# NightShade99/Self-Supervised-Vision

Hardware: NVIDIA B200
Metric: ntxent_fwd_bwd_samples_per_s (higher is better)
Workload: dtype f16

## Files before the change

### self-supervised-vision_b200/csrc/common.cuh

```cuda
#pragma once
#include <cuda.h>
#include <cuda_runtime.h>
#include <cuda_bf16.h>
#include <stdint.h>

#define SSVB_LOG2E 1.4426950408889634f
#define SSVB_LN2 0.6931471805599453f

namespace ssvb {

__device__ __forceinline__ uint32_t smem_u32(const void* p) {
  return static_cast<uint32_t>(__cvta_generic_to_shared(p));
}
__device__ __forceinline__ float ex2f(float x) {
  float y;
  asm("ex2.approx.ftz.f32 %0, %1;" : "=f"(y) : "f"(x));
  return y;
}
__device__ __forceinline__ float lg2f(float x) {
  float y;
  asm("lg2.approx.ftz.f32 %0, %1;" : "=f"(y) : "f"(x));
  return y;
}
__device__ __forceinline__ uint32_t pack_bf16x2(float lo, float hi) {
// ... 183 lines not shown
               "n"(NCOLS)
               : "memory");
  asm volatile("tcgen05.relinquish_alloc_permit.cta_group::1.sync.aligned;" ::: "memory");
}
template <int NCOLS>
__device__ __forceinline__ void tmem_dealloc(uint32_t taddr) {
  asm volatile("tcgen05.dealloc.cta_group::1.sync.aligned.b32 %0, %1;" ::"r"(taddr), "n"(NCOLS) : "memory");
}
__device__ __forceinline__ void tc_fence_before() {
  asm volatile("tcgen05.fence::before_thread_sync;" ::: "memory");
}
__device__ __forceinline__ void tc_fence_after() {
  asm volatile("tcgen05.fence::after_thread_sync;" ::: "memory");
}
__device__ __forceinline__ void umma_commit(uint64_t* bar) {
  asm volatile("tcgen05.commit.cta_group::1.mbarrier::arrive::one.shared::cluster.b64 [%0];" ::"r"(smem_u32(bar))
               : "memory");
}

__device__ __forceinline__ uint64_t make_smem_desc(uint32_t saddr, uint32_t lbo_bytes, uint32_t sbo_bytes) {
  uint64_t d = 0;
  d |= static_cast<uint64_t>((saddr & 0x3FFFFu) >> 4);
  d |= static_cast<uint64_t>((lbo_bytes >> 4) & 0x3FFFu) << 16;
  d |= static_cast<uint64_t>((sbo_bytes >> 4) & 0x3FFFu) << 32;
  d |= static_cast<uint64_t>(1) << 46;
  d |= static_cast<uint64_t>(2) << 61;
  return d;
}
__device__ __forceinline__ uint64_t desc_kmajor(uint32_t saddr) { return make_smem_desc(saddr, 16, 1024); }
__device__ __forceinline__ uint64_t desc_mnmajor(uint32_t saddr, uint32_t lbo_bytes) {
  return make_smem_desc(saddr, lbo_bytes, 1024);
}

__host__ __device__ constexpr uint32_t make_idesc(int M, int N, int a_mn_major, int b_mn_major, int ab_fmt = 1) {
  return (1u << 4) | (static_cast<uint32_t>(ab_fmt) << 7) | (static_cast<uint32_t>(ab_fmt) << 10) |
         (static_cast<uint32_t>(a_mn_major) << 15) |
         (static_cast<uint32_t>(b_mn_major) << 16) | (static_cast<uint32_t>(N >> 3) << 17) |
         (static_cast<uint32_t>(M >> 4) << 24);
}

__device__ __forceinline__ void umma_ss(uint32_t d_tmem, uint64_t adesc, uint64_t bdesc, uint32_t idesc,
                                        uint32_t accumulate) {
  asm volatile(
      "{\n\t.reg .pred p;\n\tsetp.ne.b32 p, %4, 0;\n\t"
      "tcgen05.mma.cta_group::1.kind::f16 [%0], %1, %2, %3, p;\n\t}\n"
      ::"r"(d_tmem), "l"(adesc), "l"(bdesc), "r"(idesc), "r"(accumulate)
      : "memory");
}
__device__ __forceinline__ void umma_ts(uint32_t d_tmem, uint32_t a_tmem, uint64_t bdesc, uint32_t idesc,
                                        uint32_t accumulate) {
  asm volatile(
      "{\n\t.reg .pred p;\n\tsetp.ne.b32 p, %4, 0;\n\t"
      "tcgen05.mma.cta_group::1.kind::f16 [%0], [%1], %2, %3, p;\n\t}\n"
      ::"r"(d_tmem), "r"(a_tmem), "l"(bdesc), "r"(idesc), "r"(accumulate)
      : "memory");
}

__device__ __forceinline__ void tmem_ld_x32(uint32_t taddr, uint32_t (&v)[32]) {
  asm volatile(
      "tcgen05.ld.sync.aligned.32x32b.x32.b32 "
      "{%0, %1, %2, %3, %4, %5, %6, %7, %8, %9, %10, %11, %12, %13, %14, %15, "
      "%16, %17, %18, %19, %20, %21, %22, %23, %24, %25, %26, %27, %28, %29, %30, %31}, [%32];"
      : "=r"(v[0]), "=r"(v[1]), "=r"(v[2]), "=r"(v[3]), "=r"(v[4]), "=r"(v[5]), "=r"(v[6]), "=r"(v[7]),
        "=r"(v[8]), "=r"(v[9]), "=r"(v[10]), "=r"(v[11]), "=r"(v[12]), "=r"(v[13]), "=r"(v[14]), "=r"(v[15]),
        "=r"(v[16]), "=r"(v[17]), "=r"(v[18]), "=r"(v[19]), "=r"(v[20]), "=r"(v[21]), "=r"(v[22]), "=r"(v[23]),
        "=r"(v[24]), "=r"(v[25]), "=r"(v[26]), "=r"(v[27]), "=r"(v[28]), "=r"(v[29]), "=r"(v[30]), "=r"(v[31])
      : "r"(taddr)
      : "memory");
}
__device__ __forceinline__ void tmem_ld_wait() { asm volatile("tcgen05.wait::ld.sync.aligned;" ::: "memory"); }
__device__ __forceinline__ void tmem_st_x16(uint32_t taddr, const uint32_t (&v)[16]) {
  asm volatile(
      "tcgen05.st.sync.aligned.32x32b.x16.b32 [%0], "
      "{%1, %2, %3, %4, %5, %6, %7, %8, %9, %10, %11, %12, %13, %14, %15, %16};"
      ::"r"(taddr), "r"(v[0]), "r"(v[1]), "r"(v[2]), "r"(v[3]), "r"(v[4]), "r"(v[5]), "r"(v[6]), "r"(v[7]),
        "r"(v[8]), "r"(v[9]), "r"(v[10]), "r"(v[11]), "r"(v[12]), "r"(v[13]), "r"(v[14]), "r"(v[15])
      : "memory");
}
__device__ __forceinline__ void tmem_st_wait() { asm volatile("tcgen05.wait::st.sync.aligned;" ::: "memory"); }

__device__ __forceinline__ void pdl_wait() { asm volatile("griddepcontrol.wait;" ::: "memory"); }
__device__ __forceinline__ void pdl_launch_dependents() { asm volatile("griddepcontrol.launch_dependents;" ::: "memory"); }

__device__ __forceinline__ void red_add_v4(float* addr, float a, float b, float c, float d) {
  asm volatile("red.global.add.v4.f32 [%0], {%1, %2, %3, %4};" ::"l"(addr), "f"(a), "f"(b), "f"(c), "f"(d)
               : "memory");
}

}
```

### self-supervised-vision_b200/csrc/ntxent.cu

```cuda
#include "sim_host.cuh"

using namespace ssvb;

namespace {

struct NtxPlan {
  int64_t n_glob, m, mpad, d, dpad;
  int mode;
  int normalize;
  float c, shift;
  float prescale;
  float wscale;
  float pos_c;
};

int make_plan(NtxPlan& pl, int64_t n_glob, int64_t d, int normalize, float temperature) {
  if (n_glob <= 0 || d <= 0 || !(temperature > 0.f)) return SSVB_ERR_INVALID;
  if (d % 4) return SSVB_ERR_ALIGNMENT;
  if (d > 256) return SSVB_ERR_UNSUPPORTED;
  if (2 * n_glob > (1 << 30)) return SSVB_ERR_UNSUPPORTED;
  pl.n_glob = n_glob;
  pl.m = 2 * n_glob;
  pl.mpad = sim_mpad(pl.m);
  pl.d = d;
// ... 163 lines not shown

int ssvb_ntxent_fwd(const float* zi, const float* zj, int64_t n, int64_t d, int64_t ld_zi, int64_t ld_zj,
                    int normalize, float temperature, float* loss, void* saved, void* workspace,
                    size_t workspace_bytes, void* stream) {
  SSVB_TRY(check_device_sm100());
  NtxPlan pl;
  SSVB_TRY(make_plan(pl, n, d, normalize, temperature));
  SSVB_TRY(check_rows(zi, ld_zi));
  SSVB_TRY(check_rows(zj, ld_zj));
  if (!loss || !saved || !workspace) return SSVB_ERR_INVALID;
  if (workspace_bytes < ssvb_ntxent_workspace_bytes(n, d)) return SSVB_ERR_WORKSPACE;
  cudaStream_t s = static_cast<cudaStream_t>(stream);
  SavedLayout sv = saved_layout(saved, pl.mpad, pl.dpad);
  WsLayout ws = ws_layout(workspace, pl.m, ceil_div(pl.m, 128), pl.m, pl.dpad);

  if (pl.mpad > pl.m)
    SSVB_CUDA(cudaMemsetAsync(sv.zhat + pl.m * pl.dpad, 0, (pl.mpad - pl.m) * pl.dpad * sizeof(__nv_bfloat16), s));
  {
    const int wpb = 8;
    pair_prep_kernel<<<static_cast<unsigned>(ceil_div(n, wpb)), wpb * 32, 0, s>>>(
        zi, zj, static_cast<int>(n), static_cast<int>(d), ld_zi, ld_zj, normalize, normalize ? 1 : 0, sv.zhat,
        sv.zhat + n * pl.dpad,
        static_cast<int>(pl.dpad), sv.inv_norm, sv.inv_norm + n, ws.pos, ws.pos + n, -1, pl.prescale, ws.counter);
    SSVB_LAUNCH_CHECK();
  }
  SimParams p;
  fill_sim_params_rows(p, pl, 1, pl.m, 0, 0);
  p.part_m = ws.part_m;
  p.part_l = ws.part_l;
  p.part_stride = static_cast<int>(round_up(pl.m, 256));
  int nparts;
  if (pl.mode == SIM_NTX_FIXED && pl.dpad <= 128) {
    const int ncol = plan_sym(p);
    p.colpart = ws.part_l + static_cast<size_t>(4 * p.nchunks) * p.part_stride;
    nparts = 4 * p.nchunks + ncol;
    SSVB_TRY(launch_sim_fwd_sym(sv.zhat, pl.mpad, pl.dpad, p, s));
  } else {
    plan_chunks(p, sim_fwd_bn(pl.dpad), sim_fwd_min_tiles(pl.dpad));
    nparts = 4 * p.nchunks;
    SSVB_TRY(launch_sim_fwd(pl.mode, sv.zhat, pl.mpad, sv.zhat, pl.mpad, pl.dpad, p, s));
  }
  {
    const unsigned grid = static_cast<unsigned>(ceil_div(pl.m, 256));
    const float scale = 1.f / static_cast<float>(pl.m);
    if (pl.mode == SIM_NTX_FIXED)
      lse_finalize_kernel<SIM_NTX_FIXED><<<grid, 256, 0, s>>>(ws.part_m, ws.part_l, nparts, p.part_stride,
                                                            static_cast<int>(pl.m), ws.pos, pl.c, pl.shift,
                                                            sv.stat, nullptr, ws.block_sums, ws.counter, scale, loss,
                                                            nullptr, nullptr, 0, 0, pl.wscale);
    else
      lse_finalize_kernel<SIM_NTX_ONLINE><<<grid, 256, 0, s>>>(ws.part_m, ws.part_l, nparts, p.part_stride,
                                                             static_cast<int>(pl.m), ws.pos, pl.c, pl.shift,
                                                             sv.stat, nullptr, ws.block_sums, ws.counter, scale, loss);
    SSVB_LAUNCH_CHECK();
    if (pl.mpad > pl.m) {
      const float padv = pl.mode == SIM_NTX_FIXED ? 0.f : 1e30f;
      fill_kernel<<<static_cast<unsigned>(ceil_div(pl.mpad - pl.m, 256)), 256, 0, s>>>(sv.stat + pl.m,
                                                                                       pl.mpad - pl.m, padv);
      SSVB_LAUNCH_CHECK();
    }
  }
  return SSVB_OK;
}

int ssvb_ntxent_bwd(const float* zi, const float* zj, int64_t n, int64_t d, int64_t ld_zi, int64_t ld_zj,
                    int normalize, float temperature, const float* grad_out, const void* saved, float* dzi,
                    float* dzj, int64_t ld_dzi, int64_t ld_dzj, void* workspace, size_t workspace_bytes,
                    void* stream) {
  SSVB_TRY(check_device_sm100());
  NtxPlan pl;
  SSVB_TRY(make_plan(pl, n, d, normalize, temperature));
  SSVB_TRY(check_rows(zi, ld_zi));
  SSVB_TRY(check_rows(zj, ld_zj));
  SSVB_TRY(check_rows(dzi, ld_dzi));
  SSVB_TRY(check_rows(dzj, ld_dzj));
  if (!grad_out || !saved || !workspace) return SSVB_ERR_INVALID;
  if (workspace_bytes < ssvb_ntxent_workspace_bytes(n, d)) return SSVB_ERR_WORKSPACE;
  cudaStream_t s = static_cast<cudaStream_t>(stream);
  SavedLayout sv = saved_layout(const_cast<void*>(saved), pl.mpad, pl.dpad);
  WsLayout ws = ws_layout(workspace, pl.m, ceil_div(pl.m, 128), pl.m, pl.dpad);

  SimParams p;
  fill_sim_params_rows(p, pl, 1, pl.m, 0, 0);
  plan_chunks(p, 128, 8);
  p.rowstat = sv.stat;
  p.colstat = sv.stat;
  p.dacc = ws.dacc;
  p.ld_dacc = static_cast<int>(pl.dpad);
  p.use_atomic = p.nchunks > 1;
  if (p.use_atomic) SSVB_CUDA(cudaMemsetAsync(ws.dacc, 0, pl.m * pl.dpad * sizeof(float), s));
  SSVB_TRY(launch_sim_bwd(pl.mode, sv.zhat, pl.mpad, sv.zhat, pl.mpad, pl.dpad, p, s));
  {
    const int wpb = 8;
    ntx_grad_finish_kernel<<<static_cast<unsigned>(ceil_div(pl.m, wpb)), wpb * 32, 0, s>>>(
        zi, zj, ld_zi, ld_zj, static_cast<int>(n), static_cast<int>(d), 0, ws.dacc,
        static_cast<int>(pl.dpad), sv.zhat, static_cast<int>(pl.dpad), sv.inv_norm, normalize,
        1.f / (static_cast<float>(pl.m) * temperature), grad_out, dzi, dzj, ld_dzi, ld_dzj,
        1.f / (pl.wscale * pl.prescale), 1.f / pl.prescale);
    SSVB_LAUNCH_CHECK();
  }
  return SSVB_OK;
}

size_t ssvb_ntxent_dist_workspace_bytes(int64_t world, int64_t n_local, int64_t d) {
  if (world <= 0 || n_local <= 0 || d <= 0) return 0;
  return ws_layout(nullptr, 2 * n_local, ceil_div(2 * n_local, 128), 2 * n_local * world, sim_dpad(d)).bytes;
}

namespace {
int dist_check(int64_t world, int64_t rank, int64_t n_local) {
  if (world <= 0 || rank < 0 || rank >= world || n_local <= 0) return SSVB_ERR_INVALID;
  return SSVB_OK;
}
}

int ssvb_ntxent_dist_prep(const float* zi, const float* zj, int64_t n_local, int64_t d, int64_t ld_zi,
                          int64_t ld_zj, int normalize, float temperature, int64_t world, int64_t rank,
                          void* zhat_all, float* inv_norm_local, float* pos_local, void* stream) {
  SSVB_TRY(check_device_sm100());
  SSVB_TRY(dist_check(world, rank, n_local));
  NtxPlan pl;
  SSVB_TRY(make_plan(pl, n_local * world, d, normalize, temperature));
  SSVB_TRY(check_rows(zi, ld_zi));
  SSVB_TRY(check_rows(zj, ld_zj));
  if (!zhat_all || !inv_norm_local || !pos_local) return SSVB_ERR_INVALID;
  cudaStream_t s = static_cast<cudaStream_t>(stream);
  __nv_bfloat16* zh = static_cast<__nv_bfloat16*>(zhat_all);
  if (pl.mpad > pl.m)
    SSVB_CUDA(cudaMemsetAsync(zh + pl.m * pl.dpad, 0, (pl.mpad - pl.m) * pl.dpad * sizeof(__nv_bfloat16), s));
  const int64_t row0 = rank * 2 * n_local;
  const int wpb = 8;
  pair_prep_kernel<<<static_cast<unsigned>(ceil_div(n_local, wpb)), wpb * 32, 0, s>>>(
      zi, zj, static_cast<int>(n_local), static_cast<int>(d), ld_zi, ld_zj, normalize, normalize ? 1 : 0,
      zh + row0 * pl.dpad,
      zh + (row0 + n_local) * pl.dpad, static_cast<int>(pl.dpad), inv_norm_local, inv_norm_local + n_local,
      pos_local, pos_local + n_local, -1, pl.prescale);
  SSVB_LAUNCH_CHECK();
  return SSVB_OK;
}

namespace {
int rows_fwd_impl(const void* zhat_all, int64_t world, int64_t rank, int64_t n_local, int64_t d, int normalize,
                  float temperature, const float* pos_local, float* stat_local, float* const* peer_stat,
                  float* loss_sum, void* workspace, size_t workspace_bytes, void* stream, size_t peer_stat_off = 0,
                  uint32_t gen = 0, unsigned int* counter = nullptr);
}
int ssvb_ntxent_dist_rows_fwd(const void* zhat_all, int64_t world, int64_t rank, int64_t n_local, int64_t d,
                              int normalize, float temperature, const float* pos_local, float* stat_local,
                              float* loss_sum, void* workspace, size_t workspace_bytes, void* stream) {
  if (!stat_local) return SSVB_ERR_INVALID;
  return rows_fwd_impl(zhat_all, world, rank, n_local, d, normalize, temperature, pos_local, stat_local, nullptr,
                       loss_sum, workspace, workspace_bytes, stream);
}
namespace {
int rows_fwd_impl(const void* zhat_all, int64_t world, int64_t rank, int64_t n_local, int64_t d, int normalize,
                  float temperature, const float* pos_local, float* stat_local, float* const* peer_stat,
                  float* loss_sum, void* workspace, size_t workspace_bytes, void* stream, size_t peer_stat_off,
                  uint32_t gen, unsigned int* counter) {
  SSVB_TRY(check_device_sm100());
  SSVB_TRY(dist_check(world, rank, n_local));
  NtxPlan pl;
  SSVB_TRY(make_plan(pl, n_local * world, d, normalize, temperature));
  if (!zhat_all || !pos_local || !loss_sum || !workspace) return SSVB_ERR_INVALID;
  if (workspace_bytes < ssvb_ntxent_dist_workspace_bytes(world, n_local, d)) return SSVB_ERR_WORKSPACE;
  cudaStream_t s = static_cast<cudaStream_t>(stream);
  const int64_t lr = 2 * n_local;
  WsLayout ws = ws_layout(workspace, lr, ceil_div(lr, 128), pl.m, pl.dpad);
  if (!counter) {
    counter = ws.counter;
    SSVB_CUDA(cudaMemsetAsync(counter, 0, 16, s));
  }
  float* lse_out = stat_local;
  float* term_out = stat_local ? stat_local + lr : nullptr;
  const size_t peer_off = peer_stat_off / (gen ? sizeof(uint2) : sizeof(float)) + static_cast<size_t>(rank) * 2 * lr;
// ... 397 lines not shown
```

### self-supervised-vision_b200/csrc/sim_host.cuh

```cuda
#pragma once
#include "host_util.h"
#include "sim_kernels.cuh"

namespace ssvb {

inline int64_t sim_dpad(int64_t d) { return d <= 128 ? round_up(d, 64) : 256; }
inline int64_t sim_mpad(int64_t m) { return round_up(m, 256); }
inline int sim_fwd_bn(int64_t dpad) { return dpad > 128 ? 128 : kFwdBN; }
inline int sim_fwd_min_tiles(int64_t dpad) { return 1024 / sim_fwd_bn(dpad); }

inline void plan_chunks_tiles(SimParams& p, int col_tiles, int min_tiles) {
  p.col_tiles = col_tiles;
  const int sms = num_sms();
  const int max_ch = p.col_tiles / min_tiles > 1 ? p.col_tiles / min_tiles : 1;
  int best = 1;
  double best_score = -1.0;
  for (int nch = 1; nch <= max_ch && nch <= 256; ++nch) {
    const int tpc = static_cast<int>(ceil_div(p.col_tiles, nch));
    const int real = static_cast<int>(ceil_div(p.col_tiles, tpc));
    if (real != nch) continue;
    const int64_t units = static_cast<int64_t>(p.row_blocks) * nch;
    const int64_t waves = ceil_div(units, sms);
    const double eff = static_cast<double>(p.row_blocks) * p.col_tiles / (static_cast<double>(waves) * sms * tpc);
    const double score = eff - 0.002 * nch;
    if (score > best_score) {
      best_score = score;
      best = nch;
    }
  }
  p.tiles_per_chunk = static_cast<int>(ceil_div(p.col_tiles, best));
  p.nchunks = static_cast<int>(ceil_div(p.col_tiles, p.tiles_per_chunk));
}
inline void plan_chunks(SimParams& p, int BN, int min_tiles) {
  plan_chunks_tiles(p, static_cast<int>(ceil_div(p.cols, BN)), min_tiles);
}
inline int plan_sym(SimParams& p) {
  p.band = p.row_blocks / 2 + 1;
  plan_chunks_tiles(p, (p.band + 1) / 2, sim_fwd_min_tiles(128));
  return (p.row_blocks - 1) / 2;
}

template <int KB>
int launch_sim_fwd_sym_t(const CUtensorMap& tmA, const CUtensorMap& tmB, const SimParams& p, cudaStream_t s) {
  auto kern = sim_fwd_sym_kernel<KB, true>;
  constexpr int smem = SymCfg<KB>::SMEM;
  SSVB_TRY((set_smem_once<sim_fwd_sym_kernel<KB, true>>(smem)));
  const int nunits = p.row_blocks * p.nchunks;
  const int grid = nunits < num_sms() ? nunits : num_sms();
  const int slot = prof_begin(PROF_SIM_FWD, s);
  kern<<<grid, 640, smem, s>>>(tmA, tmB, p);
  prof_end(slot, s);
  SSVB_LAUNCH_CHECK();
  return SSVB_OK;
}
inline int launch_sim_fwd_sym(const void* Z, int64_t z_rows, int64_t dpad, const SimParams& p, cudaStream_t s) {
  if (!p.opf16 || dpad > 128) return SSVB_ERR_UNSUPPORTED;
  CUtensorMap tm;
  SSVB_TRY(make_tmap_bf16(&tm, Z, z_rows, dpad, dpad, 128, true));
  return dpad == 64 ? launch_sim_fwd_sym_t<1>(tm, tm, p, s) : launch_sim_fwd_sym_t<2>(tm, tm, p, s);
}

template <int KB, int MODE, bool OPF16 = false>
int launch_sim_fwd_t(const CUtensorMap& tmA, const CUtensorMap& tmB, const SimParams& p, cudaStream_t s) {
  auto kern = sim_fwd_kernel<KB, MODE, OPF16>;
  constexpr int smem = FwdCfg<KB>::SMEM;
  SSVB_TRY((set_smem_once<sim_fwd_kernel<KB, MODE, OPF16>>(smem)));
  const int nunits = p.row_blocks * p.nchunks;
  const int grid = nunits < num_sms() ? nunits : num_sms();
  const int slot = prof_begin(PROF_SIM_FWD, s);
  kern<<<grid, 640, smem, s>>>(tmA, tmB, p);
  prof_end(slot, s);
  SSVB_LAUNCH_CHECK();
  return SSVB_OK;
}
template <int KB, int MODE, bool OPF16 = false>
int launch_sim_bwd_t(const CUtensorMap& tmA, const CUtensorMap& tmB, const SimParams& p, cudaStream_t s) {
  auto kern = sim_bwd_kernel<KB, MODE, OPF16>;
  constexpr int smem = BwdCfg<KB>::SMEM;
  SSVB_TRY((set_smem_once<sim_bwd_kernel<KB, MODE, OPF16>>(smem)));
  const int nunits = p.row_blocks * p.nchunks;
  const int grid = nunits < num_sms() ? nunits : num_sms();
  const int slot = prof_begin(PROF_SIM_BWD, s);
  kern<<<grid, 640, smem, s>>>(tmA, tmB, p);
  prof_end(slot, s);
  SSVB_LAUNCH_CHECK();
  return SSVB_OK;
}

inline int launch_sim_fwd(int mode, const void* A, int64_t a_rows, const void* B, int64_t b_rows, int64_t dpad,
                          const SimParams& p, cudaStream_t s) {
  CUtensorMap tmA, tmB;
  SSVB_TRY(make_tmap_bf16(&tmA, A, a_rows, dpad, dpad, 128, p.opf16 != 0));
  SSVB_TRY(make_tmap_bf16(&tmB, B, b_rows, dpad, dpad, sim_fwd_bn(dpad), p.opf16 != 0));
  const int KB = static_cast<int>(dpad / 64);
#define SSVB_DISPATCH(KBV)                                                      \
  switch (mode) {                                                               \
    case SIM_NTX_FIXED:                                                         \
      if (p.opf16) return launch_sim_fwd_t<KBV, SIM_NTX_FIXED, true>(tmA, tmB, p, s);                   \
      return launch_sim_fwd_t<KBV, SIM_NTX_FIXED, false>(tmA, tmB, p, s);                               \
    case SIM_NTX_ONLINE:                                                        \
      if (p.opf16) return launch_sim_fwd_t<KBV, SIM_NTX_ONLINE, true>(tmA, tmB, p, s);                  \
      return launch_sim_fwd_t<KBV, SIM_NTX_ONLINE, false>(tmA, tmB, p, s);                              \
    case SIM_MOCO: return launch_sim_fwd_t<KBV, SIM_MOCO>(tmA, tmB, p, s);      \
    default: return SSVB_ERR_INVALID;                                           \
  }
  if (KB == 1) { SSVB_DISPATCH(1) }
  if (KB == 2) { SSVB_DISPATCH(2) }
  if (KB == 4) { SSVB_DISPATCH(4) }
#undef SSVB_DISPATCH
  return SSVB_ERR_UNSUPPORTED;
}
inline int launch_sim_bwd_half(int mode, const void* A, int64_t a_rows, const void* B, int64_t b_rows, int64_t dpad,
                               const SimParams& p, cudaStream_t s);
inline int launch_sim_bwd(int mode, const void* A, int64_t a_rows, const void* B, int64_t b_rows, int64_t dpad,
                          const SimParams& p, cudaStream_t s) {
  if (dpad <= 128) return launch_sim_bwd_half(mode, A, a_rows, B, b_rows, dpad, p, s);
  SimParams q = p;
  for (int h = 0; h < 2; ++h) {
    q.dhalf = h;
    SSVB_TRY(launch_sim_bwd_half(mode, A, a_rows, B, b_rows, dpad, q, s));
  }
  return SSVB_OK;
}
inline int launch_sim_bwd_half(int mode, const void* A, int64_t a_rows, const void* B, int64_t b_rows, int64_t dpad,
                          const SimParams& p, cudaStream_t s) {
  CUtensorMap tmA, tmB;
  SSVB_TRY(make_tmap_bf16(&tmA, A, a_rows, dpad, dpad, 128, p.opf16 != 0));
  SSVB_TRY(make_tmap_bf16(&tmB, B, b_rows, dpad, dpad, 128, p.opf16 != 0));
  const int KB = static_cast<int>(dpad / 64);
#define SSVB_DISPATCH(KBV)                                                      \
  switch (mode) {                                                               \
    case SIM_NTX_FIXED:                                                         \
      if (p.opf16) return launch_sim_bwd_t<KBV, SIM_NTX_FIXED, true>(tmA, tmB, p, s);  \
      return launch_sim_bwd_t<KBV, SIM_NTX_FIXED, false>(tmA, tmB, p, s);              \
    case SIM_NTX_ONLINE:                                                        \
      if (p.opf16) return launch_sim_bwd_t<KBV, SIM_NTX_ONLINE, true>(tmA, tmB, p, s); \
      return launch_sim_bwd_t<KBV, SIM_NTX_ONLINE, false>(tmA, tmB, p, s);             \
    case SIM_MOCO: return launch_sim_bwd_t<KBV, SIM_MOCO>(tmA, tmB, p, s);      \
    default: return SSVB_ERR_INVALID;                                           \
  }
  if (KB == 1) { SSVB_DISPATCH(1) }
  if (KB == 2) { SSVB_DISPATCH(2) }
  if (KB == 4) { SSVB_DISPATCH(4) }
#undef SSVB_DISPATCH
  return SSVB_ERR_UNSUPPORTED;
}

static __global__ void pair_prep_kernel(const float* __restrict__ xi, const float* __restrict__ xj, int n, int d,
                                 int64_t ldi, int64_t ldj, int normalize, int f16, __nv_bfloat16* __restrict__ out_i,
                                 __nv_bfloat16* __restrict__ out_j, int dpad, float* __restrict__ inv_i,
                                 float* __restrict__ inv_j, float* __restrict__ pos_i, float* __restrict__ pos_j,
                                 int norm_mask = -1 ,
                                 float prescale = 1.f ,
                                 unsigned int* zero_counter = nullptr ,
                                 float* zero_rows = nullptr, int zero_ld = 0, int zero_nrows = 0 ) {
  const int warp = (blockIdx.x * blockDim.x + threadIdx.x) >> 5, lane = threadIdx.x & 31;
  if (zero_counter && blockIdx.x == 0 && threadIdx.x < 4) zero_counter[threadIdx.x] = 0u;
  if (zero_rows && warp < zero_nrows)
    for (int k = lane * 4; k < zero_ld; k += 128)
      *reinterpret_cast<float4*>(zero_rows + static_cast<int64_t>(warp) * zero_ld + k) = make_float4(0.f, 0.f, 0.f, 0.f);
  if (warp >= n) return;
  const float* ri = xi + static_cast<int64_t>(warp) * ldi;
  const float* rj = xj + static_cast<int64_t>(warp) * ldj;
  const int nmask = norm_mask >= 0 ? norm_mask : (normalize ? 3 : 0);
  float4 a[2], b[2];
  float si = 0.f, sj = 0.f;
// ... 220 lines not shown
```

### self-supervised-vision_b200/csrc/sim_kernels.cuh

```cuda
#pragma once
#include "common.cuh"

namespace ssvb {

enum SimMode { SIM_NTX_FIXED = 0, SIM_NTX_ONLINE = 1, SIM_MOCO = 2 };

struct SimParams {
  int nseg, seg_rows, seg_start[2];
  int bps;
  int row_blocks;
  int cols;
  int col_tiles;
  int nchunks, tiles_per_chunk;
  float c;
  float shift;
  float* part_m;
  float* part_l;
  int part_stride;
  int band;
  float* colpart;
  const float* rowstat;
  const float* colstat;
  float* dacc;
  int ld_dacc;
// ... 766 lines not shown
    int gt = 0, ucount = 0;
    const uint32_t a_s_full = smem_u32(&s_full[pair]), a_s_empty = smem_u32(&s_empty[pair]);
    const uint32_t a_w_full = smem_u32(&w_full[pair]), a_w_empty = smem_u32(&w_empty[pair]);
    const uint32_t a_dz_full = smem_u32(dz_full), a_dz_empty = smem_u32(dz_empty);
    const uint32_t a_sC = smem_u32(sC) + half * 64 * 4;
    for (int u = blockIdx.x; u < nunits; u += gridDim.x, ++ucount) {
      const UnitInfo ui = decode_unit(p, u);
      const int a_glob = ui.g0 + row_l;
      const bool valid = row_l < ui.nvalid;
      float rs = 0.f;
      if (valid) rs = (MODE == SIM_MOCO) ? (p.rowstat ? p.rowstat[ui.lrow0 + row_l] : p.shift) : p.rowstat[a_glob];
      float lsum = 0.f;
      for (int t = ui.t0; t < ui.t1; ++t, ++gt) {
        if ((gt & 1) != pair) continue;
        const int st = gt % NSTAGE;
        mbar_wait_a(a_s_full, (gt >> 1) & 1);
        tc_fence_after();
        const uint32_t t_s = tmem + tlane + C::T_S + pair * BN + half * 64;
        uint32_t sv[2][32];
        tmem_ld_x32(t_s, sv[0]);
        tmem_ld_x32(t_s + 32, sv[1]);
        tmem_ld_wait_regs(sv[0]);
        tmem_ld_wait_regs(sv[1]);
        tc_fence_before();
        __syncwarp();
        if (lane == 0) mbar_arrive_a(a_s_empty);
        const int j0 = t * BN + half * 64;
        const bool special = (MODE != SIM_MOCO) ? ((j0 < ui.g0 + 128) && (j0 + 64 > ui.g0)) : (j0 + 64 > p.cols);
        const uint32_t t_w = tmem + tlane + C::T_W + pair * 64 + half * 32;
        const uint32_t cs = a_sC + st * C::CS_BYTES;
        constexpr int CSTEP = 32 * 4;
        uint32_t pk[2][16];
        if (special) {
          bwd_weights32<MODE, true, OPF16>(sv[0], pk[0], p, a_glob, j0, rs, cs, lsum);
          bwd_weights32<MODE, true, OPF16>(sv[1], pk[1], p, a_glob, j0 + 32, rs, cs + CSTEP, lsum);
        } else {
          bwd_weights32<MODE, false, OPF16>(sv[0], pk[0], p, a_glob, j0, rs, cs, lsum);
          bwd_weights32<MODE, false, OPF16>(sv[1], pk[1], p, a_glob, j0 + 32, rs, cs + CSTEP, lsum);
        }
        mbar_wait_a(a_w_empty, ((gt >> 1) & 1) ^ 1);
        tc_fence_after();
        tmem_st_x16(t_w, pk[0]);
        tmem_st_x16(t_w + 16, pk[1]);
        tmem_st_wait();
        tc_fence_before();
        __syncwarp();
        if (lane == 0) mbar_arrive_a(a_w_full);
      }
      if (MODE == SIM_MOCO && p.part_l != nullptr && valid)
        p.part_l[static_cast<size_t>(ui.ch * 4 + wgi) * p.part_stride + ui.lrow0 + row_l] = lsum;
      mbar_wait_a(a_dz_full, ucount & 1);
      tc_fence_after();
      if (DP == 128 || wgi < 2) {
        const int col0 = wgi * 32;
        uint32_t v[32];
        tmem_ld_x32(tmem + tlane + C::T_DZ + col0, v);
        tmem_ld_wait_regs(v);
        if (valid) {
          float* dst = p.dacc + static_cast<size_t>(ui.lrow0 + row_l) * p.ld_dacc + col0 + (KB > 2 ? p.dhalf * 128 : 0);
          if (p.use_atomic) {
#pragma unroll
            for (int i = 0; i < 8; ++i)
              red_add_v4(dst + 4 * i, __uint_as_float(v[4 * i]), __uint_as_float(v[4 * i + 1]),
                         __uint_as_float(v[4 * i + 2]), __uint_as_float(v[4 * i + 3]));
          } else {
#pragma unroll
            for (int i = 0; i < 8; ++i)
              reinterpret_cast<float4*>(dst)[i] =
                  make_float4(__uint_as_float(v[4 * i]), __uint_as_float(v[4 * i + 1]),
                              __uint_as_float(v[4 * i + 2]), __uint_as_float(v[4 * i + 3]));
          }
        }
      }
      tc_fence_before();
      __syncwarp();
      if (lane == 0) mbar_arrive_a(a_dz_empty);
    }
  }
  tc_fence_before();
  __syncthreads();
  if (warp == 2) tmem_dealloc<512>(tmem);
}

}
```

Baseline: 14.08 million.

## Add symmetric NT-Xent backward kernel exploiting similarity matrix symmetry

Adds a dedicated backward kernel for the fixed-shift NT-Xent case with dpad=128. Because Z·Zᵀ is symmetric, each off-diagonal block pair is computed once. The kernel derives both the row-side gradient (W·Z_B) and the transposed column-side contribution (Wᵀ·Z_A) from the same weight tile, and scatters the latter into the accumulator with vector atomics. This is meant to roughly halve the similarity GEMM and exp work in the backward pass. In exchange it always uses atomics (memset plus red.add traffic), adds a more complex warp-specialized pipeline, and only runs for f16 operands with at least 16 row blocks.

```diff
diff --git a/self-supervised-vision_b200/csrc/common.cuh b/self-supervised-vision_b200/csrc/common.cuh
--- a/self-supervised-vision_b200/csrc/common.cuh
+++ b/self-supervised-vision_b200/csrc/common.cuh
@@ -289,6 +289,9 @@
 __device__ __forceinline__ void pdl_wait() { asm volatile("griddepcontrol.wait;" ::: "memory"); }
 __device__ __forceinline__ void pdl_launch_dependents() { asm volatile("griddepcontrol.launch_dependents;" ::: "memory"); }
 
+__device__ __forceinline__ void red_add_v2(float* addr, float a, float b) {
+  asm volatile("red.global.add.v2.f32 [%0], {%1, %2};" ::"l"(addr), "f"(a), "f"(b) : "memory");
+}
 __device__ __forceinline__ void red_add_v4(float* addr, float a, float b, float c, float d) {
   asm volatile("red.global.add.v4.f32 [%0], {%1, %2, %3, %4};" ::"l"(addr), "f"(a), "f"(b), "f"(c), "f"(d)
                : "memory");
diff --git a/self-supervised-vision_b200/csrc/ntxent.cu b/self-supervised-vision_b200/csrc/ntxent.cu
--- a/self-supervised-vision_b200/csrc/ntxent.cu
+++ b/self-supervised-vision_b200/csrc/ntxent.cu
@@ -269,14 +269,22 @@
 
   SimParams p;
   fill_sim_params_rows(p, pl, 1, pl.m, 0, 0);
-  plan_chunks(p, 128, 8);
   p.rowstat = sv.stat;
   p.colstat = sv.stat;
   p.dacc = ws.dacc;
   p.ld_dacc = static_cast<int>(pl.dpad);
-  p.use_atomic = p.nchunks > 1;
+  const bool sym = pl.mode == SIM_NTX_FIXED && pl.dpad == 128 && p.row_blocks >= kSymBwdMinRowBlocks;
+  if (sym) {
+    plan_sym_bwd(p);
+  } else {
+    plan_chunks(p, 128, 8);
+    p.use_atomic = p.nchunks > 1;
+  }
   if (p.use_atomic) SSVB_CUDA(cudaMemsetAsync(ws.dacc, 0, pl.m * pl.dpad * sizeof(float), s));
-  SSVB_TRY(launch_sim_bwd(pl.mode, sv.zhat, pl.mpad, sv.zhat, pl.mpad, pl.dpad, p, s));
+  if (sym)
+    SSVB_TRY(launch_sim_bwd_sym(sv.zhat, pl.mpad, p, s));
+  else
+    SSVB_TRY(launch_sim_bwd(pl.mode, sv.zhat, pl.mpad, sv.zhat, pl.mpad, pl.dpad, p, s));
   {
     const int wpb = 8;
     ntx_grad_finish_kernel<<<static_cast<unsigned>(ceil_div(pl.m, wpb)), wpb * 32, 0, s>>>(
diff --git a/self-supervised-vision_b200/csrc/sim_host.cuh b/self-supervised-vision_b200/csrc/sim_host.cuh
--- a/self-supervised-vision_b200/csrc/sim_host.cuh
+++ b/self-supervised-vision_b200/csrc/sim_host.cuh
@@ -82,6 +82,28 @@
   const int grid = nunits < num_sms() ? nunits : num_sms();
   const int slot = prof_begin(PROF_SIM_BWD, s);
   kern<<<grid, 640, smem, s>>>(tmA, tmB, p);
+  prof_end(slot, s);
+  SSVB_LAUNCH_CHECK();
+  return SSVB_OK;
+}
+
+constexpr int kSymBwdMinRowBlocks = 16;
+inline void plan_sym_bwd(SimParams& p) {
+  p.row_blocks = (p.row_blocks + 1) / 2;
+  p.band = 2 * (p.row_blocks / 2 + 1);
+  plan_chunks_tiles(p, p.band, 8);
+  p.use_atomic = 1;
+}
+inline int launch_sim_bwd_sym(const void* Z, int64_t z_rows, const SimParams& p, cudaStream_t s) {
+  if (!p.opf16 || z_rows < 256 * static_cast<int64_t>(p.row_blocks)) return SSVB_ERR_UNSUPPORTED;
+  CUtensorMap tm;
+  SSVB_TRY(make_tmap_bf16(&tm, Z, z_rows, 128, 128, 128, true));
+  constexpr int smem = SymBwdCfg::SMEM;
+  SSVB_TRY((set_smem_once<sim_bwd_sym_kernel<2>>(smem)));
+  const int nunits = p.row_blocks * p.nchunks;
+  const int grid = nunits < num_sms() ? nunits : num_sms();
+  const int slot = prof_begin(PROF_SIM_BWD, s);
+  sim_bwd_sym_kernel<2><<<grid, 640, smem, s>>>(tm, p);
   prof_end(slot, s);
   SSVB_LAUNCH_CHECK();
   return SSVB_OK;
diff --git a/self-supervised-vision_b200/csrc/sim_kernels.cuh b/self-supervised-vision_b200/csrc/sim_kernels.cuh
--- a/self-supervised-vision_b200/csrc/sim_kernels.cuh
+++ b/self-supervised-vision_b200/csrc/sim_kernels.cuh
@@ -872,4 +872,319 @@
   if (warp == 2) tmem_dealloc<512>(tmem);
 }
 
-}
+struct SymBwdCfg {
+  static constexpr int T_BYTES = 128 * 128 * 2;
+  static constexpr int CS_BYTES = 128 * 4;
+  static constexpr int NSTAGE = 3;
+  static constexpr int NBARS = 13 + 2 * NSTAGE;
+  static constexpr int SMEM = 1024 + 4 * T_BYTES + NSTAGE * (T_BYTES + CS_BYTES) + NBARS * 8 + 16;
+  static constexpr int T_DZ = 0;
+  static constexpr int T_M = 256;
+  static constexpr int T_S = 384;
+};
+static_assert(SymBwdCfg::SMEM <= 227 * 1024, "symmetric backward: shared memory");
+
+struct SymBwdUnit {
+  int I, t0, t1;
+};
+__device__ __forceinline__ SymBwdUnit decode_sym_bwd_unit(const SimParams& p, int u) {
+  SymBwdUnit su;
+  su.I = u / p.nchunks;
+  su.t0 = (u - su.I * p.nchunks) * p.tiles_per_chunk;
+  su.t1 = min(p.band, su.t0 + p.tiles_per_chunk);
+  return su;
+}
+__device__ __forceinline__ int sym_bwd_col_block(const SimParams& p, int I, int t) {
+  return 2 * ((I + (t >> 1)) % p.row_blocks) + (t & 1);
+}
+__device__ __forceinline__ bool sym_bwd_full(const SimParams& p, int t) {
+  const int o = t >> 1;
+  return o >= 1 && 2 * o < p.row_blocks;
+}
+
+__device__ __forceinline__ void red_add_row64(float* dst, const uint32_t (&v)[2][32]) {
+#pragma unroll
+  for (int h = 0; h < 2; ++h)
+#pragma unroll
+    for (int i = 0; i < 8; ++i)
+      red_add_v4(dst + h * 32 + 4 * i, __uint_as_float(v[h][4 * i]), __uint_as_float(v[h][4 * i + 1]),
+                 __uint_as_float(v[h][4 * i + 2]), __uint_as_float(v[h][4 * i + 3]));
+}
+
+template <int KB>
+__global__ void __launch_bounds__(640, 1)
+sim_bwd_sym_kernel(const __grid_constant__ CUtensorMap tmZ, const SimParams p) {
+  static_assert(KB == 2, "symmetric backward: dpad = 128");
+  using C = SymBwdCfg;
+  constexpr int NSTAGE = C::NSTAGE, TB = C::T_BYTES;
+  extern __shared__ uint8_t smem_raw[];
+  uint8_t* smem = align1024(smem_raw);
+  uint8_t* sA = smem;
+  uint8_t* sW = smem + 2 * TB;
+  uint8_t* sB = smem + 4 * TB;
+  uint8_t* sC = sB + NSTAGE * TB;
+  uint64_t* bars = reinterpret_cast<uint64_t*>(sC + NSTAGE * C::CS_BYTES);
+  uint64_t* a_full = bars;
+  uint64_t* a_empty = bars + 1;
+  uint64_t* b_full = bars + 2;
+  uint64_t* b_empty = b_full + NSTAGE;
+  uint64_t* s_full = b_empty + NSTAGE;
+  uint64_t* s_empty = s_full + 2;
+  uint64_t* w_full = s_empty + 1;
+  uint64_t* w_empty = w_full + 2;
+  uint64_t* m_full = w_empty + 2;
+  uint64_t* m_empty = m_full + 1;
+  uint64_t* dz_full = m_empty + 1;
+  uint64_t* dz_empty = dz_full + 1;
+  uint32_t* tmem_slot = reinterpret_cast<uint32_t*>(dz_empty + 1);
+
+  const int warp = threadIdx.x >> 5, lane = threadIdx.x & 31;
+  if (warp == 0 && lane == 0) tma_prefetch_desc(&tmZ);
+  if (warp == 1 && lane == 0) {
+    mbar_init(a_full, 1);
+    mbar_init(a_empty, 1);
+    for (int i = 0; i < NSTAGE; ++i) {
+      mbar_init(&b_full[i], 1);
+      mbar_init(&b_empty[i], 1);
+    }
+    for (int i = 0; i < 2; ++i) {
+      mbar_init(&s_full[i], 1);
+      mbar_init(&w_full[i], 8);
+      mbar_init(&w_empty[i], 2);
+    }
+    mbar_init(s_empty, 8);
+    mbar_init(m_full, 1);
+    mbar_init(m_empty, 16);
+    mbar_init(dz_full, 1);
+    mbar_init(dz_empty, 16);
+    fence_barrier_init();
+  }
+  if (warp == 2) tmem_alloc<512>(tmem_slot);
+  tc_fence_before();
+  __syncthreads();
+  tc_fence_after();
+  const uint32_t tmem = *tmem_slot;
+  const int nunits = p.row_blocks * p.nchunks;
+
+  if (warp < 4) {
+    asm volatile("setmaxnreg.dec.sync.aligned.u32 40;");
+    int ucount = 0, cb = 0;
+    if (warp == 0) {
+      for (int u = blockIdx.x; u < nunits; u += gridDim.x, ++ucount) {
+        const SymBwdUnit su = decode_sym_bwd_unit(p, u);
+        mbar_wait(a_empty, (ucount & 1) ^ 1);
+        if (elect_one()) {
+          mbar_expect_tx(a_full, 2 * TB);
+#pragma unroll
+          for (int b = 0; b < 2; ++b)
+#pragma unroll
+            for (int kb = 0; kb < 2; ++kb)
+              tma_load_2d(sA + b * TB + kb * (TB / 2), &tmZ, a_full, kb * 64, (2 * su.I + b) * 128);
+        }
+        __syncwarp();
+        for (int t = su.t0; t < su.t1; ++t, ++cb) {
+          const int st = cb % NSTAGE;
+          const int j = sym_bwd_col_block(p, su.I, t);
+          mbar_wait(&b_empty[st], ((cb / NSTAGE) & 1) ^ 1);
+          if (elect_one()) {
+            mbar_expect_tx(&b_full[st], TB + C::CS_BYTES);
+#pragma unroll
+            for (int kb = 0; kb < 2; ++kb) tma_load_2d(sB + st * TB + kb * (TB / 2), &tmZ, &b_full[st], kb * 64, j * 128);
+            bulk_load_1d(sC + st * C::CS_BYTES, p.colstat + j * 128, C::CS_BYTES, &b_full[st]);
+          }
+          __syncwarp();
+        }
+      }
+    } else if (warp == 1) {
+      constexpr uint32_t IDESC_S = make_idesc(128, 128, 0, 0, 0);
+      for (int u = blockIdx.x; u < nunits; u += gridDim.x, ++ucount) {
+        const SymBwdUnit su = decode_sym_bwd_unit(p, u);
+        mbar_wait(a_full, ucount & 1);
+        for (int t = su.t0; t < su.t1; ++t, ++cb) {
+          const int st = cb % NSTAGE;
+          mbar_wait(&b_full[st], (cb / NSTAGE) & 1);
+#pragma unroll
+          for (int pr = 0; pr < 2; ++pr) {
+            mbar_wait(s_empty, (pr & 1) ^ 1);
+            tc_fence_after();
+            if (elect_one()) {
+              const uint32_t abase = smem_u32(sA + pr * TB), bbase = smem_u32(sB + st * TB);
+#pragma unroll
+              for (int k = 0; k < 8; ++k)
+                umma_ss(tmem + C::T_S, desc_kmajor(abase + (k >> 2) * (TB / 2) + (k & 3) * 32),
+                        desc_kmajor(bbase + (k >> 2) * (TB / 2) + (k & 3) * 32), IDESC_S, k != 0);
+              umma_commit(&s_full[pr]);
+            }
+            __syncwarp();
+          }
+        }
+      }
+    } else if (warp == 2) {
+      constexpr uint32_t IDESC_R = make_idesc(128, 128, 0, 1, 0);
+      for (int u = blockIdx.x; u < nunits; u += gridDim.x, ++ucount) {
+        const SymBwdUnit su = decode_sym_bwd_unit(p, u);
+        mbar_wait(dz_empty, (ucount & 1) ^ 1);
+        for (int t = su.t0; t < su.t1; ++t, ++cb) {
+          const int st = cb % NSTAGE;
+#pragma unroll
+          for (int pr = 0; pr < 2; ++pr) {
+            mbar_wait(&w_full[pr], cb & 1);
+            tc_fence_after();
+            if (elect_one()) {
+              const uint32_t wbase = smem_u32(sW + pr * TB), bbase = smem_u32(sB + st * TB);
+#pragma unroll
+              for (int k = 0; k < 8; ++k)
+                umma_ss(tmem + C::T_DZ + pr * 128, desc_kmajor(wbase + (k >> 2) * (TB / 2) + (k & 3) * 32),
+                        desc_mnmajor(bbase + k * (16 * 128), TB / 2), IDESC_R, (t > su.t0 || k > 0) ? 1u : 0u);
+              umma_commit(&w_empty[pr]);
+              if (pr == 1) {
+                umma_commit(&b_empty[st]);
+                if (t == su.t1 - 1) umma_commit(dz_full);
+              }
+            }
+            __syncwarp();
+          }
+        }
+      }
+    } else {
+      constexpr uint32_t IDESC_M = make_idesc(128, 128, 1, 1, 0);
+      int fcnt = 0;
+      for (int u = blockIdx.x; u < nunits; u += gridDim.x, ++ucount) {
+        const SymBwdUnit su = decode_sym_bwd_unit(p, u);
+        for (int t = su.t0; t < su.t1; ++t, ++cb) {
+          const bool full = sym_bwd_full(p, t);
+#pragma unroll
+          for (int pr = 0; pr < 2; ++pr) {
+            mbar_wait(&w_full[pr], cb & 1);
+            if (full && pr == 0) mbar_wait(m_empty, (fcnt & 1) ^ 1);
+            tc_fence_after();
+            if (elect_one()) {
+              if (full) {
+                const uint32_t wbase = smem_u32(sW + pr * TB), abase = smem_u32(sA + pr * TB);
+#pragma unroll
+                for (int k = 0; k < 8; ++k)
+                  umma_ss(tmem + C::T_M, desc_mnmajor(wbase + k * (16 * 128), TB / 2),
+                          desc_mnmajor(abase + k * (16 * 128), TB / 2), IDESC_M, (pr | k) != 0);
+              }
+              umma_commit(&w_empty[pr]);
+              if (pr == 1) {
+                if (full) umma_commit(m_full);
+                if (t == su.t1 - 1) umma_commit(a_empty);
+              }
+            }
+            __syncwarp();
+          }
+          if (full) ++fcnt;
+        }
+      }
+    }
+  } else {
+    asm volatile("setmaxnreg.inc.sync.aligned.u32 104;");
+    const int wgi = (warp - 4) >> 2;
+    const int pair = wgi >> 1;
+    const int half = wgi & 1;
+    const int q = warp & 3;
+    const int row_l = q * 32 + lane;
+    const uint32_t tlane = static_cast<uint32_t>(q * 32) << 16;
+    const uint32_t a_s_full = smem_u32(&s_full[pair]), a_s_empty = smem_u32(s_empty);
+    const uint32_t a_w_full = smem_u32(&w_full[pair]), a_w_empty = smem_u32(&w_empty[pair]);
+    const uint32_t a_m_full = smem_u32(m_full), a_m_empty = smem_u32(m_empty);
+    const uint32_t a_dz_full = smem_u32(dz_full), a_dz_empty = smem_u32(dz_empty);
+    const uint32_t a_sC = smem_u32(sC) + half * 64 * 4;
+    const uint32_t w_row = smem_u32(sW + pair * TB + half * (TB / 2)) + row_l * 128;
+    int cb = 0, ucount = 0, fdr = 0;
+    int pend = -1;
+    auto drain_m = [&]() {
+      mbar_wait_a(a_m_full, fdr & 1);
+      tc_fence_after();
+      uint32_t v[32];
+#pragma unroll
+      for (int lh = 0; lh < 2; ++lh)
+        tmem_ld_16x256b_x4(tmem + (static_cast<uint32_t>(q * 32 + 16 * lh) << 16) + C::T_M + wgi * 32, v + 16 * lh);
+      tmem_ld_wait_regs(v);
+      tc_fence_before();
+      __syncwarp();
+      if (lane == 0) mbar_arrive_a(a_m_empty);
+      const int g = lane >> 2, c4 = lane & 3;
+#pragma unroll
+      for (int lh = 0; lh < 2; ++lh)
+#pragma unroll
+        for (int r = 0; r < 2; ++r) {
+          const int row = pend * 128 + q * 32 + 16 * lh + 8 * r + g;
+          if (row < p.cols) {
+            float* dst = p.dacc + static_cast<size_t>(row) * p.ld_dacc + wgi * 32 + 2 * c4;
+#pragma unroll
+            for (int k = 0; k < 4; ++k) {
+              const int idx = 16 * lh + 4 * k + 2 * r;
+              red_add_v2(dst + 8 * k, __uint_as_float(v[idx]), __uint_as_float(v[idx + 1]));
+            }
+          }
+        }
+      ++fdr;
+      pend = -1;
+    };
+    for (int u = blockIdx.x; u < nunits; u += gridDim.x, ++ucount) {
+      const SymBwdUnit su = decode_sym_bwd_unit(p, u);
+      const int i = 2 * su.I + pair;
+      const int a_glob = i * 128 + row_l;
+      const float rs = p.rowstat[a_glob];
+      float unused = 0.f;
+      for (int t = su.t0; t < su.t1; ++t, ++cb) {
+        const int st = cb % NSTAGE;
+        const int j = sym_bwd_col_block(p, su.I, t);
+        mbar_wait_a(a_s_full, cb & 1);
+        tc_fence_after();
+        const uint32_t t_s = tmem + tlane + C::T_S + half * 64;
+        uint32_t sv[2][32];
+        tmem_ld_x32(t_s, sv[0]);
+        tmem_ld_x32(t_s + 32, sv[1]);
+        tmem_ld_wait_regs(sv[0]);
+        tmem_ld_wait_regs(sv[1]);
+        tc_fence_before();
+        __syncwarp();
+        if (lane == 0) mbar_arrive_a(a_s_empty);
+        const int j0 = j * 128 + half * 64;
+        const uint32_t cs = a_sC + st * C::CS_BYTES;
+        uint32_t pk[2][16];
+        if (j == i) {
+          bwd_weights32<SIM_NTX_FIXED, true, true>(sv[0], pk[0], p, a_glob, j0, rs, cs, unused);
+          bwd_weights32<SIM_NTX_FIXED, true, true>(sv[1], pk[1], p, a_glob, j0 + 32, rs, cs + 128, unused);
+        } else {
+          bwd_weights32<SIM_NTX_FIXED, false, true>(sv[0], pk[0], p, a_glob, j0, rs, cs, unused);
+          bwd_weights32<SIM_NTX_FIXED, false, true>(sv[1], pk[1], p, a_glob, j0 + 32, rs, cs + 128, unused);
+        }
+        mbar_wait_a(a_w_empty, (cb & 1) ^ 1);
+#pragma unroll
+        for (int c = 0; c < 8; ++c) {
+          const uint32_t(&w)[16] = pk[c >> 2];
+          const int o = (c & 3) * 4;
+          asm volatile("st.shared.v4.b32 [%0], {%1, %2, %3, %4};" ::"r"(w_row + ((c ^ (row_l & 7)) << 4)),
+                       "r"(w[o]), "r"(w[o + 1]), "r"(w[o + 2]), "r"(w[o + 3])
+                       : "memory");
+        }
+        fence_proxy_async();
+        __syncwarp();
+        if (lane == 0) mbar_arrive_a(a_w_full);
+        if (pend >= 0) drain_m();
+        if (sym_bwd_full(p, t)) pend = j;
+      }
+      if (pend >= 0) drain_m();
+      mbar_wait_a(a_dz_full, ucount & 1);
+      tc_fence_after();
+      uint32_t v[2][32];
+      tmem_ld_x32(tmem + tlane + C::T_DZ + wgi * 64, v[0]);
+      tmem_ld_x32(tmem + tlane + C::T_DZ + wgi * 64 + 32, v[1]);
+      tmem_ld_wait_regs(v[0]);
+      tmem_ld_wait_regs(v[1]);
+      tc_fence_before();
+      __syncwarp();
+      if (lane == 0) mbar_arrive_a(a_dz_empty);
+      if (a_glob < p.cols) red_add_row64(p.dacc + static_cast<size_t>(a_glob) * p.ld_dacc + half * 64, v);
+    }
+  }
+  tc_fence_before();
+  __syncthreads();
+  if (warp == 2) tmem_dealloc<512>(tmem);
+}
+
+}
```

New measurement: 13.38 million, median of 6. -5.0%, worse.
